# haosulab/ActiveZero

Hardware: AMD Instinct MI355X
Metric: stereo pairs/sec (540x960, D=192) fwd+bwd (higher is better)
Workload: dtype f32; 1 GPU; configs[1]: PSMNet 540x960 (padded to 544 rows) D=192 fwd+bwd+Adam, supervised disparity loss, batch 4 per GPU; global_batch=4, height=540, width=960, maxdisp=192, parallelism=dp1

## Files before the change

activezero_amd/csrc/az_conv3d_c1.hip:

```cpp
#include "az_common.h"

#define C1_TH 8
#define C1_TW 32
#define C1_VS 36
#define C1_GP 36
typedef float c1_f2 __attribute__((ext_vector_type(2)));
#define C1_FMA2(a, b, c) __builtin_elementwise_fma(a, b, c)


#define C1F_TH 8
#define C1F_TW 16
template <int CTRL>
__device__ __forceinline__ float c1_dpp_add(float v) {
    return v + __builtin_bit_cast(float, __builtin_amdgcn_update_dpp(0, __builtin_bit_cast(int, v), CTRL, 0xf, 0xf, true));
}
__global__ void __launch_bounds__(256)
c1_fwd_kernel(float *__restrict__ out, const float *__restrict__ in, const float *__restrict__ w,
              const float *__restrict__ addend, const float *__restrict__ in_scale,
              const float *__restrict__ in_shift, int D, int H, int W, int tiles_x, int dseg) {
    constexpr int SX = C1F_TW + 2, SY = C1F_TH + 2;
    __shared__ __attribute__((aligned(16))) float slab[SY * SX * C1_VS];
    const int tx0 = (blockIdx.x % tiles_x) * C1F_TW, ty0 = (blockIdx.x / tiles_x) * C1F_TH;
    const int d0 = blockIdx.y * dseg, d1 = min(d0 + dseg, D), b = blockIdx.z;
    const int cp = threadIdx.x & 15, grp = threadIdx.x >> 4;
    const int ly = grp >> 1, lx0 = (grp & 1) * 8;
    const int oh = ty0 + ly;
    c1_f2 wp[27];
#pragma unroll
    for (int t = 0; t < 27; ++t) wp[t] = c1_f2{w[(cp * 2 + 0) * 27 + t], w[(cp * 2 + 1) * 27 + t]};
    c1_f2 a_prev[8], a_cur[8], a_next[8];
#pragma unroll
    for (int j = 0; j < 8; ++j) { a_prev[j] = c1_f2{0.f, 0.f}; a_cur[j] = c1_f2{0.f, 0.f}; a_next[j] = c1_f2{0.f, 0.f}; }
    constexpr int NQ = SY * SX * 8, NLD = (NQ + 255) / 256;
    float4 pre[NLD];
    const bool affine = in_scale != nullptr;
    float4 isc = make_float4(1.f, 1.f, 1.f, 1.f), ish = make_float4(0.f, 0.f, 0.f, 0.f);
    if (affine) {
        isc = reinterpret_cast<const float4 *>(in_scale)[threadIdx.x & 7];
        ish = reinterpret_cast<const float4 *>(in_shift)[threadIdx.x & 7];
    }
    unsigned okbits = 0;
    auto issue = [&](int id) {
        okbits = 0;
#pragma unroll
        for (int it = 0; it < NLD; ++it) {
            const int q = threadIdx.x + 256 * it, v = q >> 3, part = q & 7;
            const int sy = v / SX, sx = v - sy * SX;
            const int ih = ty0 - 1 + sy, iw = tx0 - 1 + sx;
            pre[it] = make_float4(0.f, 0.f, 0.f, 0.f);
            if (q < NQ && id >= 0 && id < D && ih >= 0 && ih < H && iw >= 0 && iw < W) {
                pre[it] = *reinterpret_cast<const float4 *>(
                    in + ((((size_t)b * D + id) * H + ih) * W + iw) * 32 + part * 4);
                okbits |= 1u << it;
            }
        }
    };
    issue(d0 - 1);
    for (int id = d0 - 1; id <= d1; ++id) {
        if (id >= 0 && id < D) {
            __syncthreads();
#pragma unroll
            for (int it = 0; it < NLD; ++it) {
                const int q = threadIdx.x + 256 * it;
                float4 v = pre[it];
                if (affine && ((okbits >> it) & 1u)) {
                    v.x = fmaxf(fmaf(v.x, isc.x, ish.x), 0.f); v.y = fmaxf(fmaf(v.y, isc.y, ish.y), 0.f);
                    v.z = fmaxf(fmaf(v.z, isc.z, ish.z), 0.f); v.w = fmaxf(fmaf(v.w, isc.w, ish.w), 0.f);
                }
                if (q < NQ) *reinterpret_cast<float4 *>(&slab[(q >> 3) * C1_VS + (q & 7) * 4]) = v;
            }
            __syncthreads();
        }
        if (id < d1) issue(id + 1);
        if (id >= 0 && id < D) {
#pragma unroll
            for (int kh = 0; kh < 3; ++kh) {
                c1_f2 r[10];
                const float *row = &slab[((ly + kh) * SX + lx0) * C1_VS + cp * 2];
#pragma unroll
                for (int i = 0; i < 10; ++i) {
                    const float2 x = *reinterpret_cast<const float2 *>(row + i * C1_VS);
                    r[i] = c1_f2{x.x, x.y};
                }
#pragma unroll
                for (int kw = 0; kw < 3; ++kw)
#pragma unroll
                    for (int j = 0; j < 8; ++j) {
                        a_next[j] = C1_FMA2(r[j + kw], wp[kh * 3 + kw], a_next[j]);
                        a_cur[j] = C1_FMA2(r[j + kw], wp[9 + kh * 3 + kw], a_cur[j]);
                        a_prev[j] = C1_FMA2(r[j + kw], wp[18 + kh * 3 + kw], a_prev[j]);
                    }
            }
        }
        const int od = id - 1;
        if (od >= d0 && od < d1) {
            float mine = 0.f;
#pragma unroll
            for (int j = 0; j < 8; ++j) {
                float v = a_prev[j][0] + a_prev[j][1];
                v = c1_dpp_add<0xB1>(v);
                v = c1_dpp_add<0x4E>(v);
                v = c1_dpp_add<0x141>(v);
                v = c1_dpp_add<0x140>(v);
                mine = (cp == j) ? v : mine;
            }
            const int ow = tx0 + lx0 + cp;
            if (cp < 8 && oh < H && ow < W) {
                const size_t o = (((size_t)b * D + od) * H + oh) * W + ow;
                out[o] = addend ? mine + addend[o] : mine;
            }
        }
#pragma unroll
        for (int j = 0; j < 8; ++j) { a_prev[j] = a_cur[j]; a_cur[j] = a_next[j]; a_next[j] = c1_f2{0.f, 0.f}; }
    }
}

__device__ __forceinline__ void c1_load_gtile(float *gt, const float *__restrict__ gout, int b,
                                              int od, int ty0, int tx0, int D, int H, int W) {
    constexpr int SX = C1_TW + 2, SY = C1_TH + 2;
    for (int q = threadIdx.x; q < 3 * SY * SX; q += 256) {
        const int sx = q % SX;
        const int r = q / SX;
        const int sy = r % SY, sd = r / SY;
        const int gd = od - 1 + sd, gh = ty0 - 1 + sy, gw = tx0 - 1 + sx;
        gt[r * C1_GP + sx] = (gd >= 0 && gd < D && gh >= 0 && gh < H && gw >= 0 && gw < W)
                                 ? gout[(((size_t)b * D + gd) * H + gh) * W + gw] : 0.f;
    }
}
__device__ __forceinline__ void c1_row6(float (&r)[6], const float *gt, int pd, int sy, int lx0) {
    const float *row = static_cast<const float *>(__builtin_assume_aligned(gt + (pd * (C1_TH + 2) + sy) * C1_GP + lx0, 16));
    const float4 a = *reinterpret_cast<const float4 *>(row);
    const float2 c = *reinterpret_cast<const float2 *>(row + 4);
    r[0] = a.x; r[1] = a.y; r[2] = a.z; r[3] = a.w; r[4] = c.x; r[5] = c.y;
}

__global__ void __launch_bounds__(256)
c1_dgrad_kernel(float *__restrict__ gin, const float *__restrict__ gout,
                const float *__restrict__ w, int D, int H, int W, int tiles_x) {
    constexpr int SY = C1_TH + 2;
    __shared__ __attribute__((aligned(16))) float gt[3 * SY * C1_GP];
    const int tx0 = (blockIdx.x % tiles_x) * C1_TW, ty0 = (blockIdx.x / tiles_x) * C1_TH;
    const int od = blockIdx.y, b = blockIdx.z;
    c1_load_gtile(gt, gout, b, od, ty0, tx0, D, H, W);
    const int cp = threadIdx.x & 15, grp = threadIdx.x >> 4;
    c1_f2 wp[27];
#pragma unroll
    for (int t = 0; t < 27; ++t) wp[t] = c1_f2{w[(cp * 2 + 0) * 27 + t], w[(cp * 2 + 1) * 27 + t]};
    __syncthreads();
#pragma unroll 1
    for (int p = 0; p < C1_TH * C1_TW / 128; ++p) {
        const int gi = p * 16 + grp, ly = gi >> 2, lx0 = (gi & 3) * 8;
        const int oh = ty0 + ly;
        c1_f2 acc[8];
#pragma unroll
        for (int j = 0; j < 8; ++j) acc[j] = c1_f2{0.f, 0.f};
#pragma unroll
        for (int kd = 0; kd < 3; ++kd)
#pragma unroll
            for (int kh = 0; kh < 3; ++kh) {
                float r[12];
                {
                    const float *row = static_cast<const float *>(__builtin_assume_aligned(
                        gt + ((2 - kd) * SY + ly + 2 - kh) * C1_GP + lx0, 16));
                    const float4 a = *reinterpret_cast<const float4 *>(row);
                    const float4 c = *reinterpret_cast<const float4 *>(row + 4);
                    const float2 e = *reinterpret_cast<const float2 *>(row + 8);
                    r[0] = a.x; r[1] = a.y; r[2] = a.z; r[3] = a.w; r[4] = c.x; r[5] = c.y; r[6] = c.z; r[7] = c.w;
                    r[8] = e.x; r[9] = e.y;
                }
#pragma unroll
                for (int kw = 0; kw < 3; ++kw) {
                    const int t = (kd * 3 + kh) * 3 + kw;
#pragma unroll
                    for (int j = 0; j < 8; ++j) {
                        const c1_f2 g2 = {r[j + 2 - kw], r[j + 2 - kw]};
                        acc[j] = C1_FMA2(g2, wp[t], acc[j]);
                    }
                }
            }
#pragma unroll
        for (int j = 0; j < 8; ++j) asm volatile("" : "+v"(acc[j]));
        if (oh < H) {
            float *dst = gin + ((((size_t)b * D + od) * H + oh) * W + tx0 + lx0) * 32 + cp * 2;
#pragma unroll
            for (int j = 0; j < 8; ++j)
                if (tx0 + lx0 + j < W) *reinterpret_cast<float2 *>(dst + j * 32) = make_float2(acc[j][0], acc[j][1]);
        }
    }
}

__global__ void __launch_bounds__(256)
c1_wgrad_kernel(float *__restrict__ gw, const float *__restrict__ in,
                const float *__restrict__ gout, const float *__restrict__ in_scale,
                const float *__restrict__ in_shift, int D, int H, int W, int tiles_x, int tiles_y,
                long long ntiles) {
    constexpr int SY = C1_TH + 2;
    __shared__ __attribute__((aligned(16))) float gt[3 * SY * C1_GP];
    __shared__ float red[864];
    for (int q = threadIdx.x; q < 864; q += 256) red[q] = 0.f;
    const int quad = threadIdx.x & 7, grp = threadIdx.x >> 3;
    const bool affine = in_scale != nullptr;
    float4 isc = make_float4(1.f, 1.f, 1.f, 1.f), ish = make_float4(0.f, 0.f, 0.f, 0.f);
    if (affine) {
        isc = reinterpret_cast<const float4 *>(in_scale)[quad];
        ish = reinterpret_cast<const float4 *>(in_shift)[quad];
    }
    c1_f2 a01[27], a23[27];
#pragma unroll
    for (int t = 0; t < 27; ++t) { a01[t] = c1_f2{0.f, 0.f}; a23[t] = c1_f2{0.f, 0.f}; }
    for (long long item = blockIdx.x; item < ntiles; item += gridDim.x) {
        long long r = item;
        const int tx0 = (int)(r % tiles_x) * C1_TW; r /= tiles_x;
        const int ty0 = (int)(r % tiles_y) * C1_TH; r /= tiles_y;
        const int od = (int)(r % D);
        const int b = (int)(r / D);
        __syncthreads();
        c1_load_gtile(gt, gout, b, od, ty0, tx0, D, H, W);
        __syncthreads();
#pragma unroll 1
        for (int p = 0; p < C1_TH * C1_TW / 128; ++p) {
            const int gi = p * 32 + grp, ly = gi >> 3, lx0 = (gi & 7) * 4;
            const int ih = ty0 + ly;
            c1_f2 x01[4], x23[4];
            const float *src = in + ((((size_t)b * D + od) * H + ih) * W + tx0 + lx0) * 32 + quad * 4;
#pragma unroll
            for (int j = 0; j < 4; ++j) {
                float4 x = make_float4(0.f, 0.f, 0.f, 0.f);
                if (ih < H && tx0 + lx0 + j < W) {
                    x = *reinterpret_cast<const float4 *>(src + j * 32);
                    if (affine) {
                        x.x = fmaxf(fmaf(x.x, isc.x, ish.x), 0.f); x.y = fmaxf(fmaf(x.y, isc.y, ish.y), 0.f);
                        x.z = fmaxf(fmaf(x.z, isc.z, ish.z), 0.f); x.w = fmaxf(fmaf(x.w, isc.w, ish.w), 0.f);
                    }
                }
                x01[j] = c1_f2{x.x, x.y}; x23[j] = c1_f2{x.z, x.w};
            }
#pragma unroll
            for (int kd = 0; kd < 3; ++kd)
#pragma unroll
                for (int kh = 0; kh < 3; ++kh) {
                    float r[6];
                    c1_row6(r, gt, 2 - kd, ly + 2 - kh, lx0);
#pragma unroll
                    for (int kw = 0; kw < 3; ++kw) {
                        const int t = (kd * 3 + kh) * 3 + kw;
#pragma unroll
                        for (int j = 0; j < 4; ++j) {
                            const c1_f2 g2 = {r[j + 2 - kw], r[j + 2 - kw]};
                            a01[t] = C1_FMA2(g2, x01[j], a01[t]);
                            a23[t] = C1_FMA2(g2, x23[j], a23[t]);
                        }
                    }
                }
        }
    }
#pragma unroll
    for (int c = 0; c < 4; ++c)
#pragma unroll
        for (int t = 0; t < 27; ++t) {
            float v = (c < 2 ? a01[t] : a23[t])[c & 1];
            v += __shfl_xor(v, 8); v += __shfl_xor(v, 16); v += __shfl_xor(v, 32);
            if ((threadIdx.x & 63) < 8) atomicAdd(&red[(quad * 4 + c) * 27 + t], v);
        }
    __syncthreads();
    for (int q = threadIdx.x; q < 864; q += 256) atomicAdd(&gw[q], red[q]);
}

static int c1_check(int B, int D, int H, int W) {
    if (!(B > 0 && D > 0 && H > 0 && W > 0)) return AZ_EINVAL;
    if (B > 65535 || D > 65535) return AZ_EUNSUPPORTED;
    return AZ_OK;
}

extern "C" int az_conv3d_c1_fwd(float *logits, const float *in, const float *w,
                                const float *addend, const float *in_scale, const float *in_shift, int B, int D,
                                int H, int W, void *stream) {
    AZ_REQUIRE_PTR(logits); AZ_REQUIRE_PTR(in); AZ_REQUIRE_PTR(w);
    if ((in_scale == nullptr) != (in_shift == nullptr)) return AZ_EINVAL;
    if (int e = c1_check(B, D, H, W)) return e;
    const int tiles_x = (W + C1F_TW - 1) / C1F_TW, tiles_y = (H + C1F_TH - 1) / C1F_TH;
    int best = 1;
    long long best_cost = -1;
    for (int nseg = 1; nseg <= D; ++nseg) {
        const int dseg = (D + nseg - 1) / nseg;
        const long long blocks = (long long)tiles_x * tiles_y * B * ((D + dseg - 1) / dseg);
        const long long cost = ((blocks + 767) / 768) * (dseg + 2);
        if (best_cost < 0 || cost < best_cost) { best_cost = cost; best = dseg; }
    }
    hipLaunchKernelGGL(c1_fwd_kernel, dim3(tiles_x * tiles_y, (D + best - 1) / best, B), dim3(256), 0,
                       az_stream(stream), logits, in, w, addend, in_scale, in_shift, D, H, W, tiles_x, best);
    return az_launch_status();
}

extern "C" int az_conv3d_c1_dgrad(float *grad_in, const float *grad_logits, const float *w,
                                  int B, int D, int H, int W, void *stream) {
    AZ_REQUIRE_PTR(grad_in); AZ_REQUIRE_PTR(grad_logits); AZ_REQUIRE_PTR(w);
    if (int e = c1_check(B, D, H, W)) return e;
    const int tiles_x = (W + C1_TW - 1) / C1_TW, tiles_y = (H + C1_TH - 1) / C1_TH;
    hipLaunchKernelGGL(c1_dgrad_kernel, dim3(tiles_x * tiles_y, D, B), dim3(256), 0,
                       az_stream(stream), grad_in, grad_logits, w, D, H, W, tiles_x);
    return az_launch_status();
}

extern "C" int az_conv3d_c1_wgrad(float *grad_w, const float *in, const float *grad_logits,
                                  const float *in_scale, const float *in_shift, int B, int D, int H, int W,
                                  void *stream) {
    AZ_REQUIRE_PTR(grad_w); AZ_REQUIRE_PTR(in); AZ_REQUIRE_PTR(grad_logits);
    if ((in_scale == nullptr) != (in_shift == nullptr)) return AZ_EINVAL;
    if (int e = c1_check(B, D, H, W)) return e;
    if (hipMemsetAsync(grad_w, 0, 864 * sizeof(float), az_stream(stream)) != hipSuccess)
        return AZ_ELAUNCH;
    const int tiles_x = (W + C1_TW - 1) / C1_TW, tiles_y = (H + C1_TH - 1) / C1_TH;
    const long long ntiles = (long long)B * D * tiles_y * tiles_x;
    const unsigned grid = (unsigned)(ntiles < 2048 ? ntiles : 2048);
    hipLaunchKernelGGL(c1_wgrad_kernel, dim3(grid), dim3(256), 0, az_stream(stream), grad_w, in,
                       grad_logits, in_scale, in_shift, D, H, W, tiles_x, tiles_y, ntiles);
    return az_launch_status();
}
```

Baseline: 47.17 pairs/s.

## Use MFMA fp32 matrix instructions for c1 conv3d dgrad and wgrad kernels

Rewrites the 32-to-1 channel conv3d data-gradient kernel to use 16x16x4 fp32 MFMA, with taps as the reduction dimension and weights broadcast per lane. The weight-gradient kernel now uses 32x32x2 fp32 MFMA, mapping channels by taps, and replaces the shuffle-reduction epilogue with a direct scatter of accumulators. Global loads for the next tile are prefetched into registers while the current tile computes, and the persistent grid drops from 2048 to 768 blocks. The aim is to move the FMA-bound inner loops onto matrix cores. In exchange it adds register pressure and padded-tap waste (28 slots for 27 taps), and its correctness depends on the MFMA lane layout being mapped right.

```diff
diff --git a/activezero_amd/csrc/az_conv3d_c1.hip b/activezero_amd/csrc/az_conv3d_c1.hip
--- a/activezero_amd/csrc/az_conv3d_c1.hip
+++ b/activezero_amd/csrc/az_conv3d_c1.hip
@@ -127,11 +127,11 @@
                                  ? gout[(((size_t)b * D + gd) * H + gh) * W + gw] : 0.f;
     }
 }
-__device__ __forceinline__ void c1_row6(float (&r)[6], const float *gt, int pd, int sy, int lx0) {
-    const float *row = static_cast<const float *>(__builtin_assume_aligned(gt + (pd * (C1_TH + 2) + sy) * C1_GP + lx0, 16));
-    const float4 a = *reinterpret_cast<const float4 *>(row);
-    const float2 c = *reinterpret_cast<const float2 *>(row + 4);
-    r[0] = a.x; r[1] = a.y; r[2] = a.z; r[3] = a.w; r[4] = c.x; r[5] = c.y;
+typedef float c1_f4 __attribute__((ext_vector_type(4)));
+typedef float c1_f16 __attribute__((ext_vector_type(16)));
+__device__ __forceinline__ int c1_tap_off(int t) {
+    const int kd = t / 9, kh = (t / 3) % 3, kw = t % 3;
+    return ((2 - kd) * (C1_TH + 2) + 2 - kh) * C1_GP + 2 - kw;
 }
 
 __global__ void __launch_bounds__(256)
@@ -142,49 +142,38 @@
     const int tx0 = (blockIdx.x % tiles_x) * C1_TW, ty0 = (blockIdx.x / tiles_x) * C1_TH;
     const int od = blockIdx.y, b = blockIdx.z;
     c1_load_gtile(gt, gout, b, od, ty0, tx0, D, H, W);
-    const int cp = threadIdx.x & 15, grp = threadIdx.x >> 4;
-    c1_f2 wp[27];
-#pragma unroll
-    for (int t = 0; t < 27; ++t) wp[t] = c1_f2{w[(cp * 2 + 0) * 27 + t], w[(cp * 2 + 1) * 27 + t]};
+    const int lane = threadIdx.x & 63, wave = threadIdx.x >> 6;
+    const int vx = lane & 15, q = lane >> 4;
+    float wa[7][2];
+    int toff[7];
+#pragma unroll
+    for (int s = 0; s < 7; ++s) {
+        const int t = 4 * s + q;
+        wa[s][0] = t < 27 ? w[vx * 27 + t] : 0.f;
+        wa[s][1] = t < 27 ? w[(vx + 16) * 27 + t] : 0.f;
+        toff[s] = c1_tap_off(min(t, 26));
+    }
     __syncthreads();
-#pragma unroll 1
-    for (int p = 0; p < C1_TH * C1_TW / 128; ++p) {
-        const int gi = p * 16 + grp, ly = gi >> 2, lx0 = (gi & 3) * 8;
-        const int oh = ty0 + ly;
-        c1_f2 acc[8];
-#pragma unroll
-        for (int j = 0; j < 8; ++j) acc[j] = c1_f2{0.f, 0.f};
-#pragma unroll
-        for (int kd = 0; kd < 3; ++kd)
-#pragma unroll
-            for (int kh = 0; kh < 3; ++kh) {
-                float r[12];
-                {
-                    const float *row = static_cast<const float *>(__builtin_assume_aligned(
-                        gt + ((2 - kd) * SY + ly + 2 - kh) * C1_GP + lx0, 16));
-                    const float4 a = *reinterpret_cast<const float4 *>(row);
-                    const float4 c = *reinterpret_cast<const float4 *>(row + 4);
-                    const float2 e = *reinterpret_cast<const float2 *>(row + 8);
-                    r[0] = a.x; r[1] = a.y; r[2] = a.z; r[3] = a.w; r[4] = c.x; r[5] = c.y; r[6] = c.z; r[7] = c.w;
-                    r[8] = e.x; r[9] = e.y;
-                }
-#pragma unroll
-                for (int kw = 0; kw < 3; ++kw) {
-                    const int t = (kd * 3 + kh) * 3 + kw;
-#pragma unroll
-                    for (int j = 0; j < 8; ++j) {
-                        const c1_f2 g2 = {r[j + 2 - kw], r[j + 2 - kw]};
-                        acc[j] = C1_FMA2(g2, wp[t], acc[j]);
-                    }
-                }
-            }
-#pragma unroll
-        for (int j = 0; j < 8; ++j) asm volatile("" : "+v"(acc[j]));
-        if (oh < H) {
-            float *dst = gin + ((((size_t)b * D + od) * H + oh) * W + tx0 + lx0) * 32 + cp * 2;
-#pragma unroll
-            for (int j = 0; j < 8; ++j)
-                if (tx0 + lx0 + j < W) *reinterpret_cast<float2 *>(dst + j * 32) = make_float2(acc[j][0], acc[j][1]);
+    c1_f4 acc[4][2];
+#pragma unroll
+    for (int g = 0; g < 4; ++g) {
+        const int base = (wave * 2 + (g >> 1)) * C1_GP + (g & 1) * 16 + vx;
+        acc[g][0] = c1_f4{0.f, 0.f, 0.f, 0.f};
+        acc[g][1] = c1_f4{0.f, 0.f, 0.f, 0.f};
+#pragma unroll
+        for (int s = 0; s < 7; ++s) {
+            const float gv = gt[base + toff[s]];
+            acc[g][0] = __builtin_amdgcn_mfma_f32_16x16x4f32(wa[s][0], gv, acc[g][0], 0, 0, 0);
+            acc[g][1] = __builtin_amdgcn_mfma_f32_16x16x4f32(wa[s][1], gv, acc[g][1], 0, 0, 0);
+        }
+    }
+#pragma unroll
+    for (int g = 0; g < 4; ++g) {
+        const int oh = ty0 + wave * 2 + (g >> 1), ow = tx0 + (g & 1) * 16 + vx;
+        if (oh < H && ow < W) {
+            float *dst = gin + ((((size_t)b * D + od) * H + oh) * W + ow) * 32 + q * 4;
+            *reinterpret_cast<float4 *>(dst) = make_float4(acc[g][0][0], acc[g][0][1], acc[g][0][2], acc[g][0][3]);
+            *reinterpret_cast<float4 *>(dst + 16) = make_float4(acc[g][1][0], acc[g][1][1], acc[g][1][2], acc[g][1][3]);
         }
     }
 }
@@ -198,70 +187,88 @@
     __shared__ __attribute__((aligned(16))) float gt[3 * SY * C1_GP];
     __shared__ float red[864];
     for (int q = threadIdx.x; q < 864; q += 256) red[q] = 0.f;
-    const int quad = threadIdx.x & 7, grp = threadIdx.x >> 3;
+    const int lane = threadIdx.x & 63, wave = threadIdx.x >> 6;
+    const int c = lane & 31, k = lane >> 5;
     const bool affine = in_scale != nullptr;
-    float4 isc = make_float4(1.f, 1.f, 1.f, 1.f), ish = make_float4(0.f, 0.f, 0.f, 0.f);
-    if (affine) {
-        isc = reinterpret_cast<const float4 *>(in_scale)[quad];
-        ish = reinterpret_cast<const float4 *>(in_shift)[quad];
-    }
-    c1_f2 a01[27], a23[27];
-#pragma unroll
-    for (int t = 0; t < 27; ++t) { a01[t] = c1_f2{0.f, 0.f}; a23[t] = c1_f2{0.f, 0.f}; }
+    const float isc = affine ? in_scale[c] : 1.f, ish = affine ? in_shift[c] : 0.f;
+    const int toff = c1_tap_off(min(c, 26));
+    c1_f16 acc0, acc1;
+#pragma unroll
+    for (int r = 0; r < 16; ++r) { acc0[r] = 0.f; acc1[r] = 0.f; }
+    constexpr int SX = C1_TW + 2, NG = (3 * SY * SX + 255) / 256;
+    struct Item { int tx0, ty0, od, b; };
+    auto decode = [&](long long r) {
+        Item it;
+        it.tx0 = (int)(r % tiles_x) * C1_TW; r /= tiles_x;
+        it.ty0 = (int)(r % tiles_y) * C1_TH; r /= tiles_y;
+        it.od = (int)(r % D);
+        it.b = (int)(r / D);
+        return it;
+    };
+    auto fetch = [&](const Item &it, float (&x)[32], float (&g)[NG], unsigned &gok) {
+        gok = 0;
+#pragma unroll
+        for (int i = 0; i < NG; ++i) {
+            const int q = min((int)threadIdx.x + 256 * i, 3 * SY * SX - 1);
+            const int sx = q % SX, r = q / SX;
+            const int gd = it.od - 1 + r / SY, gh = it.ty0 - 1 + r % SY, gx = it.tx0 - 1 + sx;
+            if (gd >= 0 && gd < D && gh >= 0 && gh < H && gx >= 0 && gx < W) gok |= 1u << i;
+            g[i] = gout[(((size_t)it.b * D + min(max(gd, 0), D - 1)) * H + min(max(gh, 0), H - 1)) * W + min(max(gx, 0), W - 1)];
+        }
+#pragma unroll
+        for (int rr = 0; rr < 2; ++rr) {
+            const int ih = min(it.ty0 + wave * 2 + rr, H - 1);
+            const float *src = in + (((size_t)it.b * D + it.od) * H + ih) * W * 32 + c;
+#pragma unroll
+            for (int s = 0; s < 16; ++s) x[rr * 16 + s] = src[(size_t)min(it.tx0 + 2 * s + k, W - 1) * 32];
+        }
+    };
+    float x[32], g[NG];
+    unsigned gok;
+    Item cur = decode(blockIdx.x);
+    fetch(cur, x, g, gok);
     for (long long item = blockIdx.x; item < ntiles; item += gridDim.x) {
-        long long r = item;
-        const int tx0 = (int)(r % tiles_x) * C1_TW; r /= tiles_x;
-        const int ty0 = (int)(r % tiles_y) * C1_TH; r /= tiles_y;
-        const int od = (int)(r % D);
-        const int b = (int)(r / D);
         __syncthreads();
-        c1_load_gtile(gt, gout, b, od, ty0, tx0, D, H, W);
+#pragma unroll
+        for (int i = 0; i < NG; ++i) {
+            const int q = threadIdx.x + 256 * i;
+            if (q < 3 * SY * SX) gt[(q / SX) * C1_GP + q % SX] = ((gok >> i) & 1u) ? g[i] : 0.f;
+        }
         __syncthreads();
-#pragma unroll 1
-        for (int p = 0; p < C1_TH * C1_TW / 128; ++p) {
-            const int gi = p * 32 + grp, ly = gi >> 3, lx0 = (gi & 7) * 4;
-            const int ih = ty0 + ly;
-            c1_f2 x01[4], x23[4];
-            const float *src = in + ((((size_t)b * D + od) * H + ih) * W + tx0 + lx0) * 32 + quad * 4;
-#pragma unroll
-            for (int j = 0; j < 4; ++j) {
-                float4 x = make_float4(0.f, 0.f, 0.f, 0.f);
-                if (ih < H && tx0 + lx0 + j < W) {
-                    x = *reinterpret_cast<const float4 *>(src + j * 32);
-                    if (affine) {
-                        x.x = fmaxf(fmaf(x.x, isc.x, ish.x), 0.f); x.y = fmaxf(fmaf(x.y, isc.y, ish.y), 0.f);
-                        x.z = fmaxf(fmaf(x.z, isc.z, ish.z), 0.f); x.w = fmaxf(fmaf(x.w, isc.w, ish.w), 0.f);
-                    }
+        float xn[32], gn[NG];
+        unsigned gnok = 0;
+        const bool more = item + gridDim.x < ntiles;
+        const Item nxt = decode(more ? item + gridDim.x : item);
+        if (more) fetch(nxt, xn, gn, gnok);
+#pragma unroll
+        for (int rr = 0; rr < 2; ++rr) {
+            const int ly = wave * 2 + rr;
+            if (cur.ty0 + ly < H) {
+                const float *grow = gt + ly * C1_GP + k + toff;
+#pragma unroll
+                for (int s = 0; s < 16; ++s) {
+                    float v = x[rr * 16 + s];
+                    if (affine) v = fmaxf(fmaf(v, isc, ish), 0.f);
+                    v = cur.tx0 + 2 * s + k < W ? v : 0.f;
+                    if (s & 1) acc1 = __builtin_amdgcn_mfma_f32_32x32x2f32(v, grow[2 * s], acc1, 0, 0, 0);
+                    else acc0 = __builtin_amdgcn_mfma_f32_32x32x2f32(v, grow[2 * s], acc0, 0, 0, 0);
                 }
-                x01[j] = c1_f2{x.x, x.y}; x23[j] = c1_f2{x.z, x.w};
-            }
-#pragma unroll
-            for (int kd = 0; kd < 3; ++kd)
-#pragma unroll
-                for (int kh = 0; kh < 3; ++kh) {
-                    float r[6];
-                    c1_row6(r, gt, 2 - kd, ly + 2 - kh, lx0);
-#pragma unroll
-                    for (int kw = 0; kw < 3; ++kw) {
-                        const int t = (kd * 3 + kh) * 3 + kw;
-#pragma unroll
-                        for (int j = 0; j < 4; ++j) {
-                            const c1_f2 g2 = {r[j + 2 - kw], r[j + 2 - kw]};
-                            a01[t] = C1_FMA2(g2, x01[j], a01[t]);
-                            a23[t] = C1_FMA2(g2, x23[j], a23[t]);
-                        }
-                    }
-                }
-        }
-    }
-#pragma unroll
-    for (int c = 0; c < 4; ++c)
-#pragma unroll
-        for (int t = 0; t < 27; ++t) {
-            float v = (c < 2 ? a01[t] : a23[t])[c & 1];
-            v += __shfl_xor(v, 8); v += __shfl_xor(v, 16); v += __shfl_xor(v, 32);
-            if ((threadIdx.x & 63) < 8) atomicAdd(&red[(quad * 4 + c) * 27 + t], v);
-        }
+            }
+        }
+        if (more) {
+#pragma unroll
+            for (int i = 0; i < 32; ++i) x[i] = xn[i];
+#pragma unroll
+            for (int i = 0; i < NG; ++i) g[i] = gn[i];
+            gok = gnok;
+            cur = nxt;
+        }
+    }
+    if (c < 27) {
+#pragma unroll
+        for (int r = 0; r < 16; ++r)
+            atomicAdd(&red[((r & 3) + 8 * (r >> 2) + 4 * k) * 27 + c], acc0[r] + acc1[r]);
+    }
     __syncthreads();
     for (int q = threadIdx.x; q < 864; q += 256) atomicAdd(&gw[q], red[q]);
 }
@@ -312,7 +319,7 @@
         return AZ_ELAUNCH;
     const int tiles_x = (W + C1_TW - 1) / C1_TW, tiles_y = (H + C1_TH - 1) / C1_TH;
     const long long ntiles = (long long)B * D * tiles_y * tiles_x;
-    const unsigned grid = (unsigned)(ntiles < 2048 ? ntiles : 2048);
+    const unsigned grid = (unsigned)(ntiles < 768 ? ntiles : 768);
     hipLaunchKernelGGL(c1_wgrad_kernel, dim3(grid), dim3(256), 0, az_stream(stream), grad_w, in,
                        grad_logits, in_scale, in_shift, D, H, W, tiles_x, tiles_y, ntiles);
     return az_launch_status();
```

Result: no change. 47.62 pairs/s (median of 6 runs) (+1.0%).
